# arkworks-rs/sumcheck

Measured on AMD Instinct MI355X. Metric: MLSumcheck prover field-ops/s (BLS12-381 Fr, nv=24), higher is better.
Workload: dtype u256 (BLS12-381 Fr, Montgomery form; integer arithmetic on 9 x 29-bit limbs); 1 GPU; BASELINE config 3: MLSumcheck prove, ListOfProducts [[0, 1, 2, 3], [4, 5, 6], [7, 8], [9]] over 10 tables, nv=24 (24 per GPU shard), BLS12-381 Fr, tables HBM-resident; nv=24, nv_per_gpu=24, tables=10, degree=4, launcher=single process, ranks_seen=1, communicator=none, round_loop=library, round_loop_reason=single GPU: no exchange

## Files before the change

### sumcheck_amd/build.py

```python
from __future__ import annotations

import os
import subprocess
import sys

HERE = os.path.dirname(os.path.abspath(__file__))
CSRC = os.path.join(HERE, "csrc")
OUT = os.path.join(HERE, "libsumcheck_hip.so")
OUT_EXP = os.path.join(HERE, "libsumcheck_hip_exp.so")
SOURCES = ["kernels_big.hip", "kernels_lag.hip", "kernels.hip", "kernels_tail.hip", "kernels_batch.hip", "kernels_batch_gkr.hip", "kernels_batch_eval.hip", "kernels_batch_rounds.hip", "kernels_wide.hip", "kernels_wide16.hip", "gkr.hip", "abi.hip", "protocol.hip", "batch.hip", "batch_rounds.hip", "comm.hip", "kernels_selftest.hip"]
HEADERS = ["fr_device.hpp", "fe_device.hpp", "f29_pack.hpp","kernel_common.hpp", "finalize_device.hpp", "batch_round.hpp", "wide_cell.hpp", "fe_mad_chain.inc", "fr_mac.inc", "fr_mul_gen.inc", "kernels.h", "host_fr.hpp", "transcript.hpp", "prover_internal.hpp", "load_factor.hpp", "wide_tree.hpp", "lag_index.hpp", "lane_sum.hpp", os.path.join("..", "..", "include", "sumcheck_hip.h")]
EXTRA = os.environ.get("SC_BUILD_EXTRA", "").split()
FLAGS = ["--offload-arch=gfx950", "-O3", "-std=c++17", "-fPIC", "-fvisibility=hidden", "-Wall", "-Wno-unused-function"]


def _stale(out: str) -> bool:
    if not os.path.exists(out):
        return True
    t = os.path.getmtime(out)
    deps = [os.path.join(CSRC, s) for s in SOURCES + HEADERS] + [os.path.abspath(__file__)]
    return any(os.path.getmtime(d) > t for d in deps if os.path.exists(d))


def _obj_stale(obj: str, src: str, cmd: list) -> bool:
    dep = obj + ".d"
    if not (os.path.exists(obj) and os.path.exists(dep)):
# ... 89 lines not shown
```

### sumcheck_amd/csrc/abi.hip

```cpp
#include "prover_internal.hpp"

static std::atomic<uint32_t> g_publish_timeout_ms{0};
std::chrono::milliseconds publish_timeout() {
    uint32_t ms = g_publish_timeout_ms.load(std::memory_order_relaxed);
    if (ms == 0) {
        const char *e = std::getenv("SC_PUBLISH_TIMEOUT_MS");
        const long v = e ? std::atol(e) : 0;
        ms = v > 0 ? (uint32_t)std::min<long>(v, 3600 * 1000L) : 20000u;
        g_publish_timeout_ms.store(ms, std::memory_order_relaxed);
    }
    return std::chrono::milliseconds(ms);
}
extern "C" int sc_set_publish_timeout_ms(uint32_t ms) {
    g_publish_timeout_ms.store(ms ? ms : 20000u, std::memory_order_relaxed);
    return SC_OK;
}
static thread_local std::string g_last_error;
static thread_local int g_device = 0;

static std::recursive_mutex g_gate_mutex[64];
thread_local uint16_t g_gate_depth[64];
void gate_lock(int device) {
    g_gate_mutex[(unsigned)device & 63u].lock();
    ++g_gate_depth[(unsigned)device & 63u];
// ... 53 lines not shown

int resident_quiesce(sc_prover *p);
void prover_destroy(sc_prover *p) {
    if (!p) return;
    (void)resident_quiesce(p);
    DeviceGate gate_(p->device);
    (void)hipSetDevice(p->device);
    if (p->deferred_pending && p->sig) {
        __atomic_store_n(p->sig, p->sig_seq, __ATOMIC_RELEASE);
        p->deferred_pending = false;
    }
    if (p->own_stream) (void)hipStreamSynchronize(p->own_stream);
    if (p->arena) (void)hipFree(p->arena);
    if (p->d_partials) (void)hipFree(p->d_partials);
    if (p->d_lag_area) (void)hipFree(p->d_lag_area);
    if (p->d_partials2) (void)hipFree(p->d_partials2);
    if (p->d_fin_counters) (void)hipFree(p->d_fin_counters);
    if (p->d_finprods) (void)hipFree(p->d_finprods);
    if (p->d_W) (void)hipFree(p->d_W);
    if (p->d_scratch) (void)hipFree(p->d_scratch);
    if (p->d_sums[0]) (void)hipFree(p->d_sums[0]);
    if (p->d_out) (void)hipFree(p->d_out);
    if (p->h_out) (void)hipHostFree(p->h_out);
    if (p->h_flag) (void)hipHostFree(p->h_flag);
    for (int q = 0; q < 2; ++q) {
        if (p->ring[q]) (void)hipFree(p->ring[q]);
        if (p->ev_copied[q]) (void)hipEventDestroy(p->ev_copied[q]);
        if (p->ev_consumed[q]) (void)hipEventDestroy(p->ev_consumed[q]);
    }
    if (p->d_chunk_msg) (void)hipFree(p->d_chunk_msg);
// ... 931 lines not shown
        old = g_pool.h;
        g_pool.h = nullptr;
    }
    if (old) prover_destroy(old);
}

namespace {
struct PolicyDef {
    const char *name;
    int64_t def, lo, hi;
};
constexpr PolicyDef kPolicyDefs[scd::kPolCount] = {
    {"pipeline", 1, 0, 1},     {"resident", 1, 0, 1},          {"tail_slices", 1, 0, 1}, {"vram_mailbox", 1, 0, 1},           {"wide_tree", 1, 0, 1},
    {"rccl_direct", 1, 0, 1},  {"shard_gather_log2", 15, 1, 15}, {"gkr_direct", 1, 0, 1},  {"wait_spins", 1 << 22, 1, 0xffffffffLL}, {"tail", 1, 0, 1},
    {"staged_init", 1, 0, 1},  {"batch", 1, 0, 2},        {"lag_single", 2, 0, scd::kLagMaxSkip},
};
struct PolicyTable {
    std::atomic<int64_t> v[scd::kPolCount];
    PolicyTable() {
        for (int i = 0; i < scd::kPolCount; ++i) {
            int64_t x = kPolicyDefs[i].def;
#ifdef SC_EXPERIMENTS
            std::string env = "SC_";
            for (const char *c = kPolicyDefs[i].name; *c; ++c) env += (char)std::toupper((unsigned char)*c);
            if (const char *e = std::getenv(env.c_str())) x = std::min(std::max<int64_t>(std::atoll(e), kPolicyDefs[i].lo), kPolicyDefs[i].hi);
#endif
            v[i].store(x, std::memory_order_relaxed);
        }
    }
};
// ... 288 lines not shown
```

### sumcheck_amd/csrc/kernels.h

```cpp
#pragma once
#include <hip/hip_runtime.h>
#include <stdint.h>

#include "lag_index.hpp"
#include "lane_sum.hpp"

namespace scd {

constexpr int kMaxFusedM = 8;
constexpr int kMaxSmallTables = 32;
constexpr uint64_t kSmallRoundPairs = 1u << 14;

struct FrHost {
    uint64_t l[4];
};

constexpr int32_t kNodeInf = 0x7fffffff;
__host__ __device__ constexpr int32_t node_value(int s) {
    return s == 0 ? 0 : s == 1 ? 1 : s == 2 ? kNodeInf : ((s - 3) % 2 == 0 ? -((s - 3) / 2 + 1) : ((s - 3) / 2 + 2));
}

struct BindConst {
    int32_t R[9][9];
};
// ... 31 lines not shown
    uint64_t w_off[kMaxRoundProds];
    const uint4 *Wm;
    uint4 *partials2;
    uint32_t *counters;
    uint4 *out;
    uint64_t *out_wide;
    uint4 *h_out;
    uint32_t *h_flag;
    uint32_t seq;
};
struct RoundArgs {
    TreeProd prod[kMaxRoundProds];
    int n_prod;
    RoundFin fin;
    uint32_t part_stride, part_block0;
    uint32_t binding;
};

struct FinProd {
    uint32_t M;
    uint32_t pad;
    uint64_t partial_off;
    uint64_t w_off;
};

struct TablePtrs {
    const uint4 *src[kMaxSmallTables];
    uint4 *dst[kMaxSmallTables];
    uint8_t src_f29[kMaxSmallTables];
};
// ... 168 lines not shown

enum PolicyKey {
    kPolPipeline = 0,
    kPolResident,
    kPolTailSlices,
    kPolVramMailbox,
    kPolWideTree,
    kPolRcclDirect,
    kPolShardGatherLog2,
    kPolGkrDirect,
    kPolWaitSpins,
    kPolTail,
    kPolStagedInit,
    kPolBatch,
    kPolLagSingle,
    kPolCount
};
int64_t policy(int key);

enum Plan {
    kPlanBigMergedRound1 = 0,
    kPlanBigMergedBindChain,
    kPlanBigMergedBind,
    kPlanBigClaimIdentity,
    kPlanBigF29Store,
    kPlanBigCanonicalStore,
    kPlanBigPerProductTree,
    kPlanBigWide,
    kPlanBigWide16,
    kPlanBigGeneric,
// ... 127 lines not shown
```

### sumcheck_amd/csrc/kernels_big.hip

```cpp
#include "kernel_common.hpp"
#include "finalize_device.hpp"
#include "load_factor.hpp"

#include <algorithm>
#include <cstdlib>
#include <cstring>

namespace scd {

#ifdef SC_EXPERIMENTS
template <int M>
__global__ __launch_bounds__(kBlock) void k_prod_round(const ProdArgs A, const FrHost r_h, const uint64_t n_pairs,
                                                       uint4 *__restrict__ partials) {
    __shared__ uint32_t sm[kBlock / 64][8];
    const FrU r = fru_from_host(r_h);
    Fr acc[M + 1];
#pragma unroll
    for (int t = 0; t <= M; ++t) acc[t] = fr_zero();

    const uint64_t stride = (uint64_t)gridDim.x * kBlock;
    for (uint64_t b = (uint64_t)blockIdx.x * kBlock + threadIdx.x; b < n_pairs; b += stride) {
        Fr prod[M + 1];
        bool first = true;
        for (int s = 0; s < A.n_slots; ++s) {
// ... 111 lines not shown
        for (int t = 0; t <= M; ++t) acc[t] = fe_carry_pass(fe_add(acc[t], prod[t]));
        if ((iter & 31u) == 31u) {
#pragma unroll
            for (int t = 0; t <= M; ++t) acc[t] = fe_from_fr(fe_to_fr(acc[t]));
        }
    }
#pragma unroll
    for (int t = 0; t <= M; ++t) {
        const Fr s = block_sum(fe_to_fr(acc[t]), sm);
        if (threadIdx.x == 0) fr_store(partials + 2 * ((uint64_t)t * gridDim.x + blockIdx.x), s);
    }
}

template <int M, bool kR1 = false, bool kChain = kChainDefault, bool kSkip1 = false>
__device__ __forceinline__ void tree_pass(const Slot *S, const int32_t (&r)[kBindLds], const uint64_t n_pairs, uint4 *__restrict__ row, uint32_t (*sm)[8],
                                          int32_t *lacc, const uint32_t part_stride = 0, uint4 *__restrict__ lag_area = nullptr, const int lag_m = 0) {
    const uint64_t pstride = part_stride ? part_stride : gridDim.x;
    static_assert(!(kSkip1 && kR1), "round 1 has no previous round to take node 1 from");
    int32_t *my = lacc + threadIdx.x;
#pragma unroll
    for (int i = 0; i < 9 * (M + 1); ++i) my[i * kBlock] = 0;
    const uint64_t stride = (uint64_t)gridDim.x * kBlock;
    uint32_t iter = 0;
    uint64_t b = (uint64_t)blockIdx.x * kBlock + threadIdx.x;
#ifdef SC_M4_PAIRS
    constexpr bool kM4Pairs = true;
#else
    constexpr bool kM4Pairs = kR1;
#endif
    if constexpr (tree_two_pairs(M, kM4Pairs)) {
        for (; b + stride < n_pairs; b += 2 * stride, ++iter) {
            Fe P[M + 1];
            const uint64_t b2 = b + stride;
            [[maybe_unused]] auto accumulate = [&](const int t, const Fe &v) {
                Fe acc;
#pragma unroll
                for (int l = 0; l < 9; ++l) acc.l[l] = my[(9 * t + l) * kBlock];
                acc = fe_add(acc, v);
                if (iter & 1u) acc = fe_carry_pass(acc);
// ... 239 lines not shown
                    x[((wave << lag_m) + (int)lag_class_hi(lane, lag_m)) * 8 + i] = cls[1].v[i];
                }
            }
            __syncthreads();
            if ((int)threadIdx.x < (1 << lag_m)) {
                const int c = threadIdx.x;
                Fr acc;
#pragma unroll
                for (int i = 0; i < 8; ++i) acc.v[i] = x[c * 8 + i];
                for (int w = 1; w < kBlock / 64; ++w) {
                    Fr o;
#pragma unroll
                    for (int i = 0; i < 8; ++i) o.v[i] = x[(((w << lag_m) + c)) * 8 + i];
                    acc = fr_add(acc, o);
                }
                fr_store(lag_area + 2 * ((uint64_t)c * gridDim.x + blockIdx.x), acc);
            }
            __syncthreads();
        }
    }
#else
#pragma unroll
    for (int t = 0; t <= M; ++t) {
        if (kSkip1 && t == 1) continue;
        Fe a;
#pragma unroll
        for (int l = 0; l < 9; ++l) a.l[l] = my[(9 * t + l) * kBlock];
        const Fr s = block_sum(fe_to_fr(a), sm);
        if (threadIdx.x == 0) fr_store(row + 2 * ((uint64_t)t * pstride), s);
    }
#endif
}

template <int M>
__global__ __launch_bounds__(kBlock) void k_prod_tree(const ProdArgs A, const BindConst r, const uint64_t n_pairs,
                                                      uint4 *__restrict__ partials) {
    __shared__ uint32_t sm[kBlock / 64][8];
    __shared__ int32_t rt[kBindLds];
    __shared__ int32_t lacc[9 * (M + 1) * kBlock];
    bind_consts_to_lds(r, rt);
    tree_pass<M>(A.slot, rt, n_pairs, partials + 2 * (uint64_t)blockIdx.x, sm, lacc);
}

#ifdef SC_EXPERIMENTS
constexpr int kTilePairs = 64;

template <int M>
__global__ __launch_bounds__(64 * (M + 1)) void k_round_tile(const ProdArgs A, const FrHost r32_h, const uint64_t n_pairs,
                                                             uint4 *__restrict__ partials) {
    constexpr int kThreads = 64 * (M + 1);
    constexpr int kEnt = 2 * kTilePairs;
    __shared__ int32_t lds[M * 9 * kEnt];
    const FeU r = feu_from_host(r32_h);
    const int tid = threadIdx.x;
    const int node_idx = tid >> 6;
    const int lane = tid & 63;
// ... 74 lines not shown
__global__ __launch_bounds__(kBlock, 3) void k_round_tree(const RoundArgs R, const BindConst r, const uint64_t n_pairs,
                                                       uint4 *__restrict__ partials) {
    __shared__ uint32_t sm[kBlock / 64][8];
    __shared__ int32_t rt[kBindLds];
    __shared__ int32_t lacc[9 * 5 * kBlock];
#ifdef SC_EXPERIMENTS
    __shared__ uint32_t role_sh;
#endif
    bind_consts_to_lds(r, rt);
    const int n = R.n_prod;
    int k = (int)((blockIdx.x & 7u) % (uint32_t)n);
    for (int i = 0; i < n; ++i) {
        const TreeProd &T = R.prod[k];
        uint4 *row = partials + 2 * (T.partial_off + (uint64_t)blockIdx.x);
        switch (T.M) {
        case 1: tree_pass<1>(T.slot, rt, n_pairs, row, sm, lacc); break;
        case 2: tree_pass<2>(T.slot, rt, n_pairs, row, sm, lacc); break;
        case 3: tree_pass<3>(T.slot, rt, n_pairs, row, sm, lacc); break;
        default: tree_pass<4>(T.slot, rt, n_pairs, row, sm, lacc); break;
        }
        if (++k == n) k = 0;
    }
#ifdef SC_EXPERIMENTS
    if (!R.fin.enabled) return;
    const uint32_t G = gridDim.x, n_groups = (G + kFinGroup - 1) / kFinGroup;
    const uint32_t g = blockIdx.x / kFinGroup, g_first = g * kFinGroup, g_size = min((uint32_t)kFinGroup, G - g_first);
    __syncthreads();
    if (threadIdx.x == 0) {
        __builtin_amdgcn_fence(__ATOMIC_RELEASE, "agent");
        const uint32_t d = __hip_atomic_fetch_add(R.fin.counters + 1 + g, 1u, __ATOMIC_RELAXED, __HIP_MEMORY_SCOPE_AGENT);
        role_sh = d == g_size - 1 ? 1u : 0u;
        if (role_sh) __builtin_amdgcn_fence(__ATOMIC_ACQUIRE, "agent");
    }
    __syncthreads();
// ... 28 lines not shown
        __hip_atomic_store(R.fin.counters + i, 0u, __ATOMIC_RELAXED, __HIP_MEMORY_SCOPE_AGENT);
    auto prod_of = [&](int q) -> FinProd {
        FinProd f;
        f.M = R.prod[q].M;
        f.pad = 0;
        f.partial_off = R.prod[q].partial_off;
        f.w_off = R.fin.w_off[q];
        return f;
    };
    finalize_body<kBlock>(prod_of, R.fin.Wm, n, R.fin.D, (int)n_groups, R.fin.partials2, reinterpret_cast<uint4 *>(lacc), R.fin.out, R.fin.out_wide,
                          R.fin.h_out, R.fin.h_flag, R.fin.seq, 1);
#endif
}
#endif

__global__ __launch_bounds__(kBlock, 3) void k_round1_tree_split(const RoundArgs R, const uint64_t n_pairs, uint4 *__restrict__ partials) {
    __shared__ uint32_t sm[kBlock / 64][8];
    __shared__ int32_t rt[kBindLds];
    __shared__ int32_t lacc[9 * 5 * kBlock];
    const TreeProd &T = R.prod[blockIdx.y];
    uint4 *row = partials + 2 * (T.partial_off + (uint64_t)R.part_block0 + (uint64_t)blockIdx.x);
#ifdef SC_NO_CHAIN_R1
    constexpr bool kC1 = false;
#else
    constexpr bool kC1 = true;
#endif
    switch (T.M) {
    case 1: tree_pass<1, true, kC1>(T.slot, rt, n_pairs, row, sm, lacc, R.part_stride, T.slot[0].dst, (int)T.lag_m); break;
    case 2: tree_pass<2, true, kC1>(T.slot, rt, n_pairs, row, sm, lacc, R.part_stride); break;
    case 3: tree_pass<3, true, kC1>(T.slot, rt, n_pairs, row, sm, lacc, R.part_stride); break;
    default: tree_pass<4, true, kC1>(T.slot, rt, n_pairs, row, sm, lacc, R.part_stride); break;
    }
}
template <bool kSkip1>
__device__ __forceinline__ void class_row(const TreeProd &T, const int32_t (&rt)[kBindLds], uint4 *__restrict__ row, uint32_t *x) {
    if (blockIdx.x != 0) {
        if (threadIdx.x == 0) {
            fr_store(row, fr_zero());
            if (!kSkip1) fr_store(row + 2 * (uint64_t)gridDim.x, fr_zero());
        }
        return;
    }
    const int m = (int)T.lag_m, done = (int)T.lag_done;
    const uint32_t G = T.lag_grid;
    uint4 *area = T.slot[0].dst;
    uint4 *tabs = area + 2 * lag_area_partials(m, G);
    const int n_cur = 1 << (m - done);
    if (done == 0) {
        const int per = kBlock >> m, c = (int)threadIdx.x / per, sub = (int)threadIdx.x % per;
        Fr acc = fr_zero();
        for (uint32_t b = (uint32_t)sub; b < G; b += (uint32_t)per) acc = fr_add(acc, fr_load(area + 2 * ((uint64_t)c * G + b)));
        for (int off = per >> 1; off >= 1; off >>= 1) acc = fr_add(acc, fr_shfl_down(acc, off));
        if (sub == 0) {
#pragma unroll
// ... 16 lines not shown
        const Fe l = fe_from_fr(lo), h = fe_from_fr(hi);
        const Fr v = fe_to_fr(fe_add(l, fe_mul_bind<kChainDefault>(fe_sub(h, l), rt)));
        fr_store(tabs + 2 * ((uint64_t)(((done + 1) & 1) << m) + threadIdx.x), v);
#pragma unroll
        for (int i = 0; i < 8; ++i) y[threadIdx.x * 8 + i] = v.v[i];
    }
    __syncthreads();
    if (threadIdx.x < 2 && !(kSkip1 && threadIdx.x == 1)) {
        Fr acc = fr_zero();
        for (int e = (int)threadIdx.x; e < n_cur / 2; e += 2) {
            Fr o;
#pragma unroll
            for (int i = 0; i < 8; ++i) o.v[i] = y[e * 8 + i];
            acc = fr_add(acc, o);
        }
        fr_store(row + 2 * ((uint64_t)threadIdx.x * gridDim.x), acc);
    }
}
template <bool kChain, bool kSkip1, bool kLag = false>
__global__ __launch_bounds__(kBlock, 3) void k_round_tree_split(const RoundArgs R, const BindConst r, const uint64_t n_pairs, uint4 *__restrict__ partials) {
    __shared__ uint32_t sm[kBlock / 64][8];
    __shared__ int32_t rt[kBindLds];
    __shared__ int32_t lacc[9 * 5 * kBlock];
    bind_consts_to_lds(r, rt);
    const TreeProd &T = R.prod[blockIdx.y];
    uint4 *row = partials + 2 * (T.partial_off + (uint64_t)blockIdx.x);
    if constexpr (kLag) {
        if (T.lag_m != 0) {
            class_row<kSkip1>(T, rt, row, reinterpret_cast<uint32_t *>(lacc));
            return;
        }
    }
    switch (T.M) {
    case 1: tree_pass<1, false, kChain, kSkip1>(T.slot, rt, n_pairs, row, sm, lacc); break;
    case 2: tree_pass<2, false, kChain, kSkip1>(T.slot, rt, n_pairs, row, sm, lacc); break;
    case 3: tree_pass<3, false, kChain, kSkip1>(T.slot, rt, n_pairs, row, sm, lacc); break;
    default: tree_pass<4, false, kChain, kSkip1>(T.slot, rt, n_pairs, row, sm, lacc); break;
    }
}

#ifdef SC_EXPERIMENTS
__global__ __launch_bounds__(kBlock, 3) void k_round1_tree(const RoundArgs R, const uint64_t n_pairs, uint4 *__restrict__ partials) {
    __shared__ uint32_t sm[kBlock / 64][8];
    __shared__ int32_t rt[kBindLds];
    __shared__ int32_t lacc[9 * 5 * kBlock];
    const int n = R.n_prod;
    int k = (int)((blockIdx.x & 7u) % (uint32_t)n);
    for (int i = 0; i < n; ++i) {
        const TreeProd &T = R.prod[k];
        uint4 *row = partials + 2 * (T.partial_off + (uint64_t)blockIdx.x);
        switch (T.M) {
        case 1: tree_pass<1, true>(T.slot, rt, n_pairs, row, sm, lacc); break;
        case 2: tree_pass<2, true>(T.slot, rt, n_pairs, row, sm, lacc); break;
        case 3: tree_pass<3, true>(T.slot, rt, n_pairs, row, sm, lacc); break;
        default: tree_pass<4, true>(T.slot, rt, n_pairs, row, sm, lacc); break;
        }
        if (++k == n) k = 0;
    }
}
#endif

#ifdef SC_EXPERIMENTS
template <int M>
static hipError_t launch_prod_round_t(const ProdArgs &args, const FrHost &r, uint64_t n_pairs, FrHost *d_partials, int grid,
                                      hipStream_t stream) {
    hipLaunchKernelGGL(k_prod_round<M>, dim3(grid), dim3(kBlock), 0, stream, args, r, n_pairs, (uint4 *)d_partials);
    return hipGetLastError();
}

#endif
// ... 61 lines not shown
#else
    (void)split;
    (void)extra_lds;
#endif
#ifdef SC_NO_CHAIN_R2
    bool canonical_sources = false;
#else
    bool canonical_sources = !round1;
#endif
    for (int q = 0; q < args.n_prod && canonical_sources; ++q)
        for (uint32_t f = 0; f < args.prod[q].M; ++f) canonical_sources = canonical_sources && args.prod[q].slot[f].src_f29 == 0;
#ifdef SC_SERIAL_EPILOGUE
    for (int q = 0; q < args.n_prod; ++q)
        if (args.prod[q].lag_m != 0) return hipErrorInvalidValue;
#endif
    const dim3 g(grid, args.n_prod), b(kBlock);
    uint4 *const part = (uint4 *)d_partials;
    plan_hit(round1 ? kPlanBigMergedRound1 : canonical_sources ? kPlanBigMergedBindChain : kPlanBigMergedBind);
    if (skip1) plan_hit(kPlanBigClaimIdentity);
    if (round1) {
        if (skip1) return hipErrorInvalidValue;
        hipLaunchKernelGGL(k_round1_tree_split, g, b, 0, stream, args, n_pairs, part);
    } else {
        bool lag = false;
        for (int q = 0; q < args.n_prod; ++q) lag = lag || args.prod[q].lag_m != 0;
        const int sel = (canonical_sources ? 4 : 0) | (skip1 ? 2 : 0) | (lag ? 1 : 0);
        switch (sel) {
        case 7: hipLaunchKernelGGL((k_round_tree_split<true, true, true>), g, b, 0, stream, args, r32, n_pairs, part); break;
        case 6: hipLaunchKernelGGL((k_round_tree_split<true, true, false>), g, b, 0, stream, args, r32, n_pairs, part); break;
        case 5: hipLaunchKernelGGL((k_round_tree_split<true, false, true>), g, b, 0, stream, args, r32, n_pairs, part); break;
        case 4: hipLaunchKernelGGL((k_round_tree_split<true, false, false>), g, b, 0, stream, args, r32, n_pairs, part); break;
// ... 58 lines not shown
```

### sumcheck_amd/csrc/protocol.hip

```cpp
#include "prover_internal.hpp"

uint64_t small_pairs_limit() {
#ifdef SC_EXPERIMENTS
    static const uint64_t v = [] {
        const char *e = std::getenv("SC_SMALL_LOG2");
        return e ? (1ULL << std::atoi(e)) : scd::kSmallRoundPairs;
    }();
    return v;
#else
    return scd::kSmallRoundPairs;
#endif
}

bool launches_are_async(sc_prover *p) {
    static const bool ok = [p] {
        uint32_t *h = nullptr, *d = nullptr;
        FrHost *dm = nullptr;
        if (hipHostMalloc(reinterpret_cast<void **>(&h), 256, hipHostMallocMapped | hipHostMallocCoherent) != hipSuccess) return false;
        bool good = hipHostGetDevicePointer(reinterpret_cast<void **>(&d), h, 0) == hipSuccess &&
                    hipMalloc(reinterpret_cast<void **>(&dm), sizeof(FrHost)) == hipSuccess;
        if (good) {
            std::memset(h, 0, 256);
            good = scd::launch_wait_challenge(d, 0xffffffffu, reinterpret_cast<const FrHost *>(d + 16), dm, p->stream, 1) == hipSuccess &&
                   hipStreamSynchronize(p->stream) == hipSuccess;
// ... 128 lines not shown
        for (uint32_t l = 0; l < k; ++l) make_bind_const(p->lag.r[l], A.r[l]);
        A.levels = k;
        A.n_groups = (1ULL << p->nv) >> 2;
        for (Table &t : p->tabs) {
            if (!t.lag) continue;
            A.src = t.cur;
            A.dst = t.buf[t.next];
            scd::plan_hit(catch_up ? scd::kPlanBigLagCatchUp : scd::kPlanBigLagMaterialize);
            HIP_TRY(scd::launch_fix_deep(A, p->use_f29, p->stream));
            t.cur = t.buf[t.next];
            t.cur_f29 = p->use_f29;
            t.next ^= 1;
        }
    }
    lag_clear(p);
    return SC_OK;
}

int launch_round_streamed(sc_prover *p, const uint64_t *r_or_null, uint64_t *d_wide, bool publish_to_host) {
    scd::plan_hit(scd::kPlanBigStreamed);
    if (p->exhausted) return sc_internal_fail(SC_ERR_NOT_ACTIVE, "Prover is not active");
    if (r_or_null && p->round == 0) return sc_internal_fail(SC_ERR_FIRST_ROUND_HAS_MSG, "first round should be prover first.");
    if (!r_or_null && p->round > 0) return sc_internal_fail(SC_ERR_MISSING_MSG, "verifier message is empty");
    sch::Fr r = sch::zero();
    if (r_or_null) {
        std::memcpy(&r, r_or_null, 32);
        if (sch::geq_p(r)) return sc_internal_fail(SC_ERR_BAD_ARG, "challenge is not a canonical field element");
    }
    HIP_TRY(hipSetDevice(p->device));
    int rc_t = collect_timing(p);
// ... 41 lines not shown
                        sl.src_f29 = 0;
                        if (!bind) {
                            sl.mode = 0;
                        } else if (!bound[u]) {
                            sl.mode = 1;
                            sl.dst = t.buf[0] + 2 * (c * (C / 2));
                            sl.dst_f29 = p->use_f29 ? 1 : 0;
                            bound[u] = 1;
                        } else {
                            sl.mode = 3;
                            sl.dst_f29 = p->use_f29 ? 1 : 0;
                        }
                    }
                }
            }
            HIP_TRY(scd::launch_round_tree(ra, rc, pairs_per_chunk, p->d_partials, grid, p->stream, true));
            if (bind) {
                for (uint32_t u = 0; u < p->U; ++u)
                    if (!bound[u]) HIP_TRY(scd::launch_fix(ring_tab(u), p->tabs[u].buf[0] + 2 * (c * (C / 2)), to_dev(r), C / 2, p->stream));
            }
        } else {
            std::vector<const uint4 *> src(p->U);
            for (uint32_t u = 0; u < p->U; ++u) {
                if (bind) {
                    uint4 *dst = p->tabs[u].buf[0] + 2 * (c * (C / 2));
                    HIP_TRY(scd::launch_fix(ring_tab(u), dst, to_dev(r), C / 2, p->stream));
                    src[u] = dst;
                } else {
                    src[u] = ring_tab(u);
                }
// ... 127 lines not shown
        for (uint32_t k = 0; k < p->K; ++k) {
            const Product &pr = p->prods[k];
            scd::TreeProd &tp = ra.prod[k];
            tp.M = pr.M;
            tp.partial_off = pr.partial_off;
            int f = 0;
            for (size_t s2 = 0; s2 < pr.tables.size(); ++s2)
                for (uint32_t rep = 0; rep < pr.exps[s2]; ++rep, ++f) {
                    tp.slot[f].exp = 1;
                    tp.slot[f].mode = 0;
                    tp.slot[f].src = p->tabs[pr.tables[s2]].buf[0] + 2 * (size_t)first;
                }
        }
        ra.part_stride = (uint32_t)G;
        ra.part_block0 = (uint32_t)block0;
        HIP_TRY(scd::launch_round_tree(ra, rc, chunk >> 1, p->d_partials, gc, p->stream, true, false));
        block0 += gc;
    }
    if (block0 != G) return sc_internal_fail(SC_ERR_HIP, "staged initialisation: the sections do not cover the grid");
    scd::plan_hit(scd::kPlanBigStagedRound1);
    const bool keeps = scd::finalize_keeps_sums((int)p->K, (int)p->D, G, !p->h_finprods.empty(), fin_mb_enabled());
    HIP_TRY(scd::launch_finalize(p->d_finprods, p->h_finprods.data(), p->d_W, (int)p->K, (int)p->D, G, p->d_partials, keeps ? p->d_sums[1] : p->d_scratch, p->d_out, nullptr,
                                 p->h_out_dev, p->h_flag_dev, p->seq + 1, 1, fin_mb_enabled() ? p->d_fin_mb_counter : nullptr, p->stream, nullptr));
    p->r1_cached = true;
    p->r1_keeps = keeps;
    return SC_OK;
}

int launch_round(sc_prover *p, const uint64_t *r_or_null, uint64_t *d_wide, bool publish_to_host, bool deferred) {
    if (p->res.active) {
// ... 291 lines not shown
        }
        p->seq += 1;
        ra.fin.enabled = p->fused_finalize ? 1 : 0;
        ra.fin.D = (int)p->D;
        for (uint32_t k = 0; k < p->K; ++k) ra.fin.w_off[k] = p->h_finprods[k].w_off;
        ra.fin.Wm = reinterpret_cast<const uint4 *>(p->d_W);
        ra.fin.partials2 = reinterpret_cast<uint4 *>(p->d_partials2);
        ra.fin.counters = p->d_fin_counters;
        ra.fin.out = reinterpret_cast<uint4 *>(p->d_out);
        ra.fin.out_wide = d_wide;
        ra.fin.h_out = publish_to_host ? reinterpret_cast<uint4 *>(p->h_out_dev) : nullptr;
        ra.fin.h_flag = publish_to_host ? p->h_flag_dev : nullptr;
        ra.fin.seq = p->seq;
        if (p->timing) HIP_TRY(hipEventRecord(p->prod_ev[0], p->stream));
        if (bind) scd::plan_hit(p->use_f29 ? scd::kPlanBigF29Store : scd::kPlanBigCanonicalStore);
        HIP_TRY(scd::launch_round_tree(ra, rc, n_pairs, p->d_partials, grid, p->stream, split, skip1));
        if (p->timing) HIP_TRY(hipEventRecord(p->prod_ev[1], p->stream));
        scaled = 1;
        if (p->fused_finalize) finalized = true;
        else p->seq -= 1;
    }
    for (uint32_t k = 0; k < p->K && !small && !merged; ++k) {
        const Product &pr = p->prods[k];
        FrHost *partials = p->d_partials + pr.partial_off;
        if (p->timing) HIP_TRY(hipEventRecord(p->prod_ev[2 * k], p->stream));
        if (pr.fused && p->kernel_variant == 3 && (pr.M <= 4 || p->wide_tree)) {
            ProdArgs a;
            std::memset(&a, 0, sizeof(a));
            a.n_slots = (int)pr.M;
            int f = 0;
// ... 990 lines not shown
```

### sumcheck_amd/csrc/prover_internal.hpp

```cpp
#pragma once
#include <hip/hip_runtime.h>

#include <dlfcn.h>
#include <rccl/rccl.h>

#include <algorithm>
#include <array>
#include <atomic>
#include <chrono>
#include <condition_variable>
#include <map>
#include <memory>
#include <mutex>
#include <cstdarg>
#include <cstdio>
#include <cstdlib>
#include <cstring>
#include <new>
#include <string>
#include <thread>
#include <vector>

#include "../../include/sumcheck_hip.h"
#include "host_fr.hpp"
// ... 86 lines not shown
    uint32_t *d_fin_counters = nullptr;
    FinProd *d_finprods = nullptr;
    FrHost *d_W = nullptr;
    uint32_t w_elems = 0;
    bool w_scaled = false;
    FrHost *d_scratch = nullptr;
    FrHost *d_sums[2] = {nullptr, nullptr};
    int64_t sums_round = -1;
    struct Lag {
        bool active = false;
        uint32_t j = 0, m = 0, grid = 0;
        std::vector<sch::Fr> r;
    } lag;
    FrHost *d_lag_area = nullptr;
    uint32_t lag_areas = 0;
    FrHost *d_out = nullptr;
    FrHost *h_out = nullptr;
    uint32_t *h_flag = nullptr;
    FrHost *h_out_dev = nullptr;
    uint32_t *h_flag_dev = nullptr;
    uint32_t seq = 0;
    uint64_t *d_wide = nullptr;
    uint32_t wide_gen = 0;
    bool wide_tagged = false;
    uint64_t *h_wide = nullptr;
    uint64_t *h_wide_dev = nullptr;
    void *d_tail_send = nullptr, *d_tail_recv = nullptr, *d_tail_tabs = nullptr;
    sc_prover *tail = nullptr;
    uint32_t tail_ranks = 0;
    size_t tail_buf_bytes = 0;
// ... 69 lines not shown
bool handle_pool_offer(sc_prover *p);
std::vector<uint8_t> pool_key_of(const sc_poly_desc *d, int device);
sc_prover *handle_pool_take(const std::vector<uint8_t> &key);
void claim_weights(uint32_t M, const sch::Fr &r, sch::Fr *lam);
void build_node_matrix(uint32_t M, uint32_t D, const sch::Fr &scale, std::vector<sch::Fr> &out);
int collect_timing(sc_prover *p);
int prover_bind_out(sc_prover *p, const uint64_t *r, uint64_t *d_out);
uint64_t sc_internal_cache_limit();
constexpr int kResidentGone = -1;
extern std::atomic<uint64_t> g_stat[8];
enum { kStatTailLaunches = 0, kStatTailSlotBusy = 1, kStatTailSlotReclaims = 2, kStatResidentStarts = 3, kStatResidentGone = 4, kStatProofRetries = 5, kStatTailSlices = 6 };
bool wide_tree_enabled();
int resident_quiesce(sc_prover *p);
int launch_round(sc_prover *p, const uint64_t *r_or_null, uint64_t *d_wide, bool publish_to_host, bool deferred = false);
int materialize_lagging(sc_prover *p, bool catch_up = false);
void lag_clear(sc_prover *p);
bool staged_init_applies(const sc_prover *p);
int staged_copy_and_round1(sc_prover *p, const uint64_t *const *host_tables);
int await_round(sc_prover *p, uint64_t *out_evals, uint32_t want);
bool wait_gave_up(sc_prover *p);
void abandon_deferred(sc_prover *p);
int sc_internal_run_rounds(sc_prover *p, sch::Blake2b512Rng &rng, uint32_t n_rounds, uint64_t *out_msgs, sch::Fr *out_challenges);
bool launches_are_async(sc_prover *p);
bool tail_slot_acquire(sc_prover *p, bool resident);
void tail_slot_release(sc_prover *p);
void sc_internal_release_batch_cache();
struct SharedMeta {
    uint32_t nv = 0, U = 0, K = 0, D = 0, max_mult = 0;
    int n_combos = 0;
    bool fits_args = false;
// ... 79 lines not shown
```

Baseline: 559.1 billion field-ops/s.

## Schedule round-tree blocks through a weighted row-order table for load balance

Replaces the 2D grid (blocks × products) of the split tree kernels with a 1D grid that reads a host-built schedule table mapping each block to a (product row, block index). Rows are ranked by estimated multiply/bind cost, and heavier rows are issued earlier by a configurable lead, so long-running product rows start first and the tail of the dispatch is filled with cheaper work. Tables are cached per prover and uploaded once. This adds a table lookup per block and a host build plus copy on first use.

Measured after the change: 561.1 billion field-ops/s, median of 6. No clear change (+0.4%).

```diff
diff --git a/sumcheck_amd/build.py b/sumcheck_amd/build.py
--- a/sumcheck_amd/build.py
+++ b/sumcheck_amd/build.py
@@ -9,7 +9,7 @@
 OUT = os.path.join(HERE, "libsumcheck_hip.so")
 OUT_EXP = os.path.join(HERE, "libsumcheck_hip_exp.so")
 SOURCES = ["kernels_big.hip", "kernels_lag.hip", "kernels.hip", "kernels_tail.hip", "kernels_batch.hip", "kernels_batch_gkr.hip", "kernels_batch_eval.hip", "kernels_batch_rounds.hip", "kernels_wide.hip", "kernels_wide16.hip", "gkr.hip", "abi.hip", "protocol.hip", "batch.hip", "batch_rounds.hip", "comm.hip", "kernels_selftest.hip"]
-HEADERS = ["fr_device.hpp", "fe_device.hpp", "f29_pack.hpp","kernel_common.hpp", "finalize_device.hpp", "batch_round.hpp", "wide_cell.hpp", "fe_mad_chain.inc", "fr_mac.inc", "fr_mul_gen.inc", "kernels.h", "host_fr.hpp", "transcript.hpp", "prover_internal.hpp", "load_factor.hpp", "wide_tree.hpp", "lag_index.hpp", "lane_sum.hpp", os.path.join("..", "..", "include", "sumcheck_hip.h")]
+HEADERS = ["fr_device.hpp", "fe_device.hpp", "f29_pack.hpp","kernel_common.hpp", "finalize_device.hpp", "batch_round.hpp", "wide_cell.hpp", "fe_mad_chain.inc", "fr_mac.inc", "fr_mul_gen.inc", "kernels.h", "host_fr.hpp", "transcript.hpp", "prover_internal.hpp", "load_factor.hpp", "wide_tree.hpp", "lag_index.hpp", "lane_sum.hpp", "row_schedule.hpp", os.path.join("..", "..", "include", "sumcheck_hip.h")]
 EXTRA = os.environ.get("SC_BUILD_EXTRA", "").split()
 FLAGS = ["--offload-arch=gfx950", "-O3", "-std=c++17", "-fPIC", "-fvisibility=hidden", "-Wall", "-Wno-unused-function"]
 
diff --git a/sumcheck_amd/csrc/abi.hip b/sumcheck_amd/csrc/abi.hip
--- a/sumcheck_amd/csrc/abi.hip
+++ b/sumcheck_amd/csrc/abi.hip
@@ -91,6 +91,8 @@
     if (p->arena) (void)hipFree(p->arena);
     if (p->d_partials) (void)hipFree(p->d_partials);
     if (p->d_lag_area) (void)hipFree(p->d_lag_area);
+    for (auto &rs : p->row_scheds)
+        if (rs.d_table) (void)hipFree(rs.d_table);
     if (p->d_partials2) (void)hipFree(p->d_partials2);
     if (p->d_fin_counters) (void)hipFree(p->d_fin_counters);
     if (p->d_finprods) (void)hipFree(p->d_finprods);
@@ -1052,6 +1054,7 @@
     {"pipeline", 1, 0, 1},     {"resident", 1, 0, 1},          {"tail_slices", 1, 0, 1}, {"vram_mailbox", 1, 0, 1},           {"wide_tree", 1, 0, 1},
     {"rccl_direct", 1, 0, 1},  {"shard_gather_log2", 15, 1, 15}, {"gkr_direct", 1, 0, 1},  {"wait_spins", 1 << 22, 1, 0xffffffffLL}, {"tail", 1, 0, 1},
     {"staged_init", 1, 0, 1},  {"batch", 1, 0, 2},        {"lag_single", 2, 0, scd::kLagMaxSkip},
+    {"row_lead_r1", 4, 0, scd::kSchedMaxLead}, {"row_lead", 4, 0, scd::kSchedMaxLead},
 };
 struct PolicyTable {
     std::atomic<int64_t> v[scd::kPolCount];
diff --git a/sumcheck_amd/csrc/kernels.h b/sumcheck_amd/csrc/kernels.h
--- a/sumcheck_amd/csrc/kernels.h
+++ b/sumcheck_amd/csrc/kernels.h
@@ -4,6 +4,7 @@
 
 #include "lag_index.hpp"
 #include "lane_sum.hpp"
+#include "row_schedule.hpp"
 
 namespace scd {
 
@@ -69,6 +70,8 @@
     int n_prod;
     RoundFin fin;
     uint32_t part_stride, part_block0;
+    const uint16_t *sched;
+    uint32_t row_blocks;
     uint32_t binding;
 };
 
@@ -267,6 +270,8 @@
     kPolStagedInit,
     kPolBatch,
     kPolLagSingle,
+    kPolRowLeadR1,
+    kPolRowLead,
     kPolCount
 };
 int64_t policy(int key);
diff --git a/sumcheck_amd/csrc/kernels_big.hip b/sumcheck_amd/csrc/kernels_big.hip
--- a/sumcheck_amd/csrc/kernels_big.hip
+++ b/sumcheck_amd/csrc/kernels_big.hip
@@ -149,15 +149,16 @@
 
 template <int M, bool kR1 = false, bool kChain = kChainDefault, bool kSkip1 = false>
 __device__ __forceinline__ void tree_pass(const Slot *S, const int32_t (&r)[kBindLds], const uint64_t n_pairs, uint4 *__restrict__ row, uint32_t (*sm)[8],
-                                          int32_t *lacc, const uint32_t part_stride = 0, uint4 *__restrict__ lag_area = nullptr, const int lag_m = 0) {
-    const uint64_t pstride = part_stride ? part_stride : gridDim.x;
+                                          int32_t *lacc, const uint32_t bx, const uint32_t nb, const uint32_t part_stride = 0, uint4 *__restrict__ lag_area = nullptr,
+                                          const int lag_m = 0) {
+    const uint64_t pstride = part_stride ? part_stride : nb;
     static_assert(!(kSkip1 && kR1), "round 1 has no previous round to take node 1 from");
     int32_t *my = lacc + threadIdx.x;
 #pragma unroll
     for (int i = 0; i < 9 * (M + 1); ++i) my[i * kBlock] = 0;
-    const uint64_t stride = (uint64_t)gridDim.x * kBlock;
+    const uint64_t stride = (uint64_t)nb * kBlock;
     uint32_t iter = 0;
-    uint64_t b = (uint64_t)blockIdx.x * kBlock + threadIdx.x;
+    uint64_t b = (uint64_t)bx * kBlock + threadIdx.x;
 #ifdef SC_M4_PAIRS
     constexpr bool kM4Pairs = true;
 #else
@@ -427,7 +428,7 @@
                     for (int i = 0; i < 8; ++i) o.v[i] = x[(((w << lag_m) + c)) * 8 + i];
                     acc = fr_add(acc, o);
                 }
-                fr_store(lag_area + 2 * ((uint64_t)c * gridDim.x + blockIdx.x), acc);
+                fr_store(lag_area + 2 * ((uint64_t)c * nb + bx), acc);
             }
             __syncthreads();
         }
@@ -452,7 +453,7 @@
     __shared__ int32_t rt[kBindLds];
     __shared__ int32_t lacc[9 * (M + 1) * kBlock];
     bind_consts_to_lds(r, rt);
-    tree_pass<M>(A.slot, rt, n_pairs, partials + 2 * (uint64_t)blockIdx.x, sm, lacc);
+    tree_pass<M>(A.slot, rt, n_pairs, partials + 2 * (uint64_t)blockIdx.x, sm, lacc, blockIdx.x, gridDim.x);
 }
 
 #ifdef SC_EXPERIMENTS
@@ -557,10 +558,10 @@
         const TreeProd &T = R.prod[k];
         uint4 *row = partials + 2 * (T.partial_off + (uint64_t)blockIdx.x);
         switch (T.M) {
-        case 1: tree_pass<1>(T.slot, rt, n_pairs, row, sm, lacc); break;
-        case 2: tree_pass<2>(T.slot, rt, n_pairs, row, sm, lacc); break;
-        case 3: tree_pass<3>(T.slot, rt, n_pairs, row, sm, lacc); break;
-        default: tree_pass<4>(T.slot, rt, n_pairs, row, sm, lacc); break;
+        case 1: tree_pass<1>(T.slot, rt, n_pairs, row, sm, lacc, blockIdx.x, gridDim.x); break;
+        case 2: tree_pass<2>(T.slot, rt, n_pairs, row, sm, lacc, blockIdx.x, gridDim.x); break;
+        case 3: tree_pass<3>(T.slot, rt, n_pairs, row, sm, lacc, blockIdx.x, gridDim.x); break;
+        default: tree_pass<4>(T.slot, rt, n_pairs, row, sm, lacc, blockIdx.x, gridDim.x); break;
         }
         if (++k == n) k = 0;
     }
@@ -619,30 +620,35 @@
 }
 #endif
 
+__device__ __forceinline__ uint32_t sched_item(const RoundArgs &R) {
+    return sched_entry_of_word(reinterpret_cast<const uint32_t *>(R.sched)[blockIdx.x >> 1], blockIdx.x);
+}
 __global__ __launch_bounds__(kBlock, 3) void k_round1_tree_split(const RoundArgs R, const uint64_t n_pairs, uint4 *__restrict__ partials) {
     __shared__ uint32_t sm[kBlock / 64][8];
     __shared__ int32_t rt[kBindLds];
     __shared__ int32_t lacc[9 * 5 * kBlock];
-    const TreeProd &T = R.prod[blockIdx.y];
-    uint4 *row = partials + 2 * (T.partial_off + (uint64_t)R.part_block0 + (uint64_t)blockIdx.x);
+    const uint32_t item = sched_item(R), nb = R.row_blocks, bx = min(sched_x(item), nb - 1u);
+    const TreeProd &T = R.prod[min(sched_row(item), (uint32_t)R.n_prod - 1u)];
+    uint4 *row = partials + 2 * (T.partial_off + (uint64_t)R.part_block0 + (uint64_t)bx);
 #ifdef SC_NO_CHAIN_R1
     constexpr bool kC1 = false;
 #else
     constexpr bool kC1 = true;
 #endif
     switch (T.M) {
-    case 1: tree_pass<1, true, kC1>(T.slot, rt, n_pairs, row, sm, lacc, R.part_stride, T.slot[0].dst, (int)T.lag_m); break;
-    case 2: tree_pass<2, true, kC1>(T.slot, rt, n_pairs, row, sm, lacc, R.part_stride); break;
-    case 3: tree_pass<3, true, kC1>(T.slot, rt, n_pairs, row, sm, lacc, R.part_stride); break;
-    default: tree_pass<4, true, kC1>(T.slot, rt, n_pairs, row, sm, lacc, R.part_stride); break;
+    case 1: tree_pass<1, true, kC1>(T.slot, rt, n_pairs, row, sm, lacc, bx, nb, R.part_stride, T.slot[0].dst, (int)T.lag_m); break;
+    case 2: tree_pass<2, true, kC1>(T.slot, rt, n_pairs, row, sm, lacc, bx, nb, R.part_stride); break;
+    case 3: tree_pass<3, true, kC1>(T.slot, rt, n_pairs, row, sm, lacc, bx, nb, R.part_stride); break;
+    default: tree_pass<4, true, kC1>(T.slot, rt, n_pairs, row, sm, lacc, bx, nb, R.part_stride); break;
     }
 }
 template <bool kSkip1>
-__device__ __forceinline__ void class_row(const TreeProd &T, const int32_t (&rt)[kBindLds], uint4 *__restrict__ row, uint32_t *x) {
-    if (blockIdx.x != 0) {
+__device__ __forceinline__ void class_row(const TreeProd &T, const int32_t (&rt)[kBindLds], uint4 *__restrict__ row, uint32_t *x, const uint32_t bx,
+                                          const uint32_t nb) {
+    if (bx != 0) {
         if (threadIdx.x == 0) {
             fr_store(row, fr_zero());
-            if (!kSkip1) fr_store(row + 2 * (uint64_t)gridDim.x, fr_zero());
+            if (!kSkip1) fr_store(row + 2 * (uint64_t)nb, fr_zero());
         }
         return;
     }
@@ -689,7 +695,7 @@
             for (int i = 0; i < 8; ++i) o.v[i] = y[e * 8 + i];
             acc = fr_add(acc, o);
         }
-        fr_store(row + 2 * ((uint64_t)threadIdx.x * gridDim.x), acc);
+        fr_store(row + 2 * ((uint64_t)threadIdx.x * nb), acc);
     }
 }
 template <bool kChain, bool kSkip1, bool kLag = false>
@@ -698,19 +704,20 @@
     __shared__ int32_t rt[kBindLds];
     __shared__ int32_t lacc[9 * 5 * kBlock];
     bind_consts_to_lds(r, rt);
-    const TreeProd &T = R.prod[blockIdx.y];
-    uint4 *row = partials + 2 * (T.partial_off + (uint64_t)blockIdx.x);
+    const uint32_t item = sched_item(R), nb = R.row_blocks, bx = min(sched_x(item), nb - 1u);
+    const TreeProd &T = R.prod[min(sched_row(item), (uint32_t)R.n_prod - 1u)];
+    uint4 *row = partials + 2 * (T.partial_off + (uint64_t)bx);
     if constexpr (kLag) {
         if (T.lag_m != 0) {
-            class_row<kSkip1>(T, rt, row, reinterpret_cast<uint32_t *>(lacc));
+            class_row<kSkip1>(T, rt, row, reinterpret_cast<uint32_t *>(lacc), bx, nb);
             return;
         }
     }
     switch (T.M) {
-    case 1: tree_pass<1, false, kChain, kSkip1>(T.slot, rt, n_pairs, row, sm, lacc); break;
-    case 2: tree_pass<2, false, kChain, kSkip1>(T.slot, rt, n_pairs, row, sm, lacc); break;
-    case 3: tree_pass<3, false, kChain, kSkip1>(T.slot, rt, n_pairs, row, sm, lacc); break;
-    default: tree_pass<4, false, kChain, kSkip1>(T.slot, rt, n_pairs, row, sm, lacc); break;
+    case 1: tree_pass<1, false, kChain, kSkip1>(T.slot, rt, n_pairs, row, sm, lacc, bx, nb); break;
+    case 2: tree_pass<2, false, kChain, kSkip1>(T.slot, rt, n_pairs, row, sm, lacc, bx, nb); break;
+    case 3: tree_pass<3, false, kChain, kSkip1>(T.slot, rt, n_pairs, row, sm, lacc, bx, nb); break;
+    default: tree_pass<4, false, kChain, kSkip1>(T.slot, rt, n_pairs, row, sm, lacc, bx, nb); break;
     }
 }
 
@@ -725,10 +732,10 @@
         const TreeProd &T = R.prod[k];
         uint4 *row = partials + 2 * (T.partial_off + (uint64_t)blockIdx.x);
         switch (T.M) {
-        case 1: tree_pass<1, true>(T.slot, rt, n_pairs, row, sm, lacc); break;
-        case 2: tree_pass<2, true>(T.slot, rt, n_pairs, row, sm, lacc); break;
-        case 3: tree_pass<3, true>(T.slot, rt, n_pairs, row, sm, lacc); break;
-        default: tree_pass<4, true>(T.slot, rt, n_pairs, row, sm, lacc); break;
+        case 1: tree_pass<1, true>(T.slot, rt, n_pairs, row, sm, lacc, blockIdx.x, gridDim.x); break;
+        case 2: tree_pass<2, true>(T.slot, rt, n_pairs, row, sm, lacc, blockIdx.x, gridDim.x); break;
+        case 3: tree_pass<3, true>(T.slot, rt, n_pairs, row, sm, lacc, blockIdx.x, gridDim.x); break;
+        default: tree_pass<4, true>(T.slot, rt, n_pairs, row, sm, lacc, blockIdx.x, gridDim.x); break;
         }
         if (++k == n) k = 0;
     }
@@ -820,7 +827,9 @@
     for (int q = 0; q < args.n_prod; ++q)
         if (args.prod[q].lag_m != 0) return hipErrorInvalidValue;
 #endif
-    const dim3 g(grid, args.n_prod), b(kBlock);
+    if (args.sched == nullptr || args.row_blocks != (uint32_t)grid || grid < 1 || grid > kSchedMaxBlocks || args.n_prod < 1 || args.n_prod > kSchedMaxRows)
+        return hipErrorInvalidValue;
+    const dim3 g((uint32_t)grid * (uint32_t)args.n_prod), b(kBlock);
     uint4 *const part = (uint4 *)d_partials;
     plan_hit(round1 ? kPlanBigMergedRound1 : canonical_sources ? kPlanBigMergedBindChain : kPlanBigMergedBind);
     if (skip1) plan_hit(kPlanBigClaimIdentity);
diff --git a/sumcheck_amd/csrc/protocol.hip b/sumcheck_amd/csrc/protocol.hip
--- a/sumcheck_amd/csrc/protocol.hip
+++ b/sumcheck_amd/csrc/protocol.hip
@@ -166,6 +166,39 @@
         }
     }
     lag_clear(p);
+    return SC_OK;
+}
+
+int prover_row_schedule(sc_prover *p, scd::RoundArgs &ra, int grid, int lead, bool skip1) {
+    const int K = ra.n_prod;
+    if (K < 1 || K > scd::kSchedMaxRows || grid < 1 || grid > scd::kSchedMaxBlocks) return sc_internal_fail(SC_ERR_HIP, "no block schedule for %d rows of %d blocks", K, grid);
+    lead = std::min(std::max(lead, 0), scd::kSchedMaxLead);
+    uint32_t w[scd::kSchedMaxRows] = {};
+    for (int q = 0; q < K; ++q) {
+        const scd::TreeProd &T = ra.prod[q];
+        int binds = 0;
+        for (uint32_t f = 0; f < T.M; ++f) binds += T.slot[f].mode != 0 ? 1 : 0;
+        w[q] = scd::sched_row_weight((int)T.M, skip1, binds, ra.binding != 0 && T.lag_m != 0);
+    }
+    ra.row_blocks = (uint32_t)grid;
+    for (const sc_prover::RowSched &rs : p->row_scheds)
+        if (rs.K == (uint32_t)K && rs.g == (uint32_t)grid && rs.lead == (uint32_t)lead && std::memcmp(rs.weight, w, sizeof(w)) == 0) {
+            ra.sched = rs.d_table;
+            return SC_OK;
+        }
+    std::vector<uint16_t> h(2 * (size_t)scd::sched_table_words(K, grid), 0);
+    if (scd::sched_build(w, K, grid, lead, h.data()) != (uint32_t)K * (uint32_t)grid) return sc_internal_fail(SC_ERR_HIP, "the block schedule was not built");
+    sc_prover::RowSched rs;
+    rs.K = (uint32_t)K, rs.g = (uint32_t)grid, rs.lead = (uint32_t)lead;
+    std::memcpy(rs.weight, w, sizeof(w));
+    HIP_TRY(hipMalloc(reinterpret_cast<void **>(&rs.d_table), h.size() * sizeof(uint16_t)));
+    const hipError_t e = hipMemcpy(rs.d_table, h.data(), h.size() * sizeof(uint16_t), hipMemcpyHostToDevice);
+    if (e != hipSuccess) {
+        (void)hipFree(rs.d_table);
+        HIP_TRY(e);
+    }
+    p->row_scheds.push_back(rs);
+    ra.sched = rs.d_table;
     return SC_OK;
 }
 
@@ -237,6 +270,7 @@
                     }
                 }
             }
+            if (int rc_s = prover_row_schedule(p, ra, grid, (int)scd::policy(bind ? scd::kPolRowLead : scd::kPolRowLeadR1), false)) return rc_s;
             HIP_TRY(scd::launch_round_tree(ra, rc, pairs_per_chunk, p->d_partials, grid, p->stream, true));
             if (bind) {
                 for (uint32_t u = 0; u < p->U; ++u)
@@ -394,6 +428,7 @@
         }
         ra.part_stride = (uint32_t)G;
         ra.part_block0 = (uint32_t)block0;
+        if (int rc_s = prover_row_schedule(p, ra, gc, scd::kSchedMaxLead, false)) return rc_s;
         HIP_TRY(scd::launch_round_tree(ra, rc, chunk >> 1, p->d_partials, gc, p->stream, true, false));
         block0 += gc;
     }
@@ -715,6 +750,8 @@
         ra.fin.seq = p->seq;
         if (p->timing) HIP_TRY(hipEventRecord(p->prod_ev[0], p->stream));
         if (bind) scd::plan_hit(p->use_f29 ? scd::kPlanBigF29Store : scd::kPlanBigCanonicalStore);
+        if (split)
+            if (int rc_s = prover_row_schedule(p, ra, grid, (int)scd::policy(bind ? scd::kPolRowLead : scd::kPolRowLeadR1), skip1)) return rc_s;
         HIP_TRY(scd::launch_round_tree(ra, rc, n_pairs, p->d_partials, grid, p->stream, split, skip1));
         if (p->timing) HIP_TRY(hipEventRecord(p->prod_ev[1], p->stream));
         scaled = 1;
diff --git a/sumcheck_amd/csrc/prover_internal.hpp b/sumcheck_amd/csrc/prover_internal.hpp
--- a/sumcheck_amd/csrc/prover_internal.hpp
+++ b/sumcheck_amd/csrc/prover_internal.hpp
@@ -124,6 +124,12 @@
     } lag;
     FrHost *d_lag_area = nullptr;
     uint32_t lag_areas = 0;
+    struct RowSched {
+        uint32_t K = 0, g = 0, lead = 0;
+        uint32_t weight[scd::kSchedMaxRows] = {};
+        uint16_t *d_table = nullptr;
+    };
+    std::vector<RowSched> row_scheds;
     FrHost *d_out = nullptr;
     FrHost *h_out = nullptr;
     uint32_t *h_flag = nullptr;
@@ -223,6 +229,7 @@
 int resident_quiesce(sc_prover *p);
 int launch_round(sc_prover *p, const uint64_t *r_or_null, uint64_t *d_wide, bool publish_to_host, bool deferred = false);
 int materialize_lagging(sc_prover *p, bool catch_up = false);
+int prover_row_schedule(sc_prover *p, scd::RoundArgs &ra, int grid, int lead, bool skip1);
 void lag_clear(sc_prover *p);
 bool staged_init_applies(const sc_prover *p);
 int staged_copy_and_round1(sc_prover *p, const uint64_t *const *host_tables);
diff --git a/sumcheck_amd/csrc/row_schedule.hpp b/sumcheck_amd/csrc/row_schedule.hpp
--- /dev/null
+++ b/sumcheck_amd/csrc/row_schedule.hpp
@@ -0,0 +1,64 @@
+#pragma once
+#include <cstdint>
+
+#if defined(__HIPCC__)
+#define SC_SCHED_FN __host__ __device__ constexpr
+#else
+#define SC_SCHED_FN constexpr
+#endif
+
+namespace scd {
+
+constexpr int kSchedMaxRows = 12;
+constexpr int kSchedMaxBlocks = 1024;
+constexpr int kSchedMaxLead = 4;
+constexpr int kSchedXBits = 10;
+constexpr uint32_t kSchedMulMads = 153, kSchedBindMads = 97;
+
+SC_SCHED_FN uint16_t sched_entry(uint32_t row, uint32_t x) { return (uint16_t)((row << kSchedXBits) | x); }
+SC_SCHED_FN uint32_t sched_row(uint32_t entry) { return entry >> kSchedXBits; }
+SC_SCHED_FN uint32_t sched_x(uint32_t entry) { return entry & ((1u << kSchedXBits) - 1u); }
+SC_SCHED_FN uint32_t sched_entry_of_word(uint32_t word, uint32_t i) { return (word >> (16u * (i & 1u))) & 0xffffu; }
+SC_SCHED_FN uint32_t sched_table_words(int K, int g) { return ((uint32_t)K * (uint32_t)g + 1u) / 2u; }
+
+SC_SCHED_FN uint32_t sched_tree_products(int M, bool skip1) {
+    const uint32_t full = M <= 1 ? 0u : M == 2 ? 3u : M == 3 ? 7u : 11u;
+    return full != 0 && skip1 ? full - 1u : full;
+}
+SC_SCHED_FN uint32_t sched_row_weight(int M, bool skip1, int bind_factors, bool class_row) {
+    return class_row ? 0u : kSchedMulMads * sched_tree_products(M, skip1) + kSchedBindMads * 2u * (uint32_t)bind_factors;
+}
+
+SC_SCHED_FN void sched_rank_rows(const uint32_t *weight, int K, uint8_t *rank) {
+    for (int a = 0; a < K; ++a) {
+        int before = 0;
+        for (int b = 0; b < K; ++b)
+            if (weight[b] > weight[a] || (weight[b] == weight[a] && b < a)) ++before;
+        rank[a] = (uint8_t)before;
+    }
+}
+
+SC_SCHED_FN uint32_t sched_key(uint32_t rank, uint32_t x, int g, int lead) { return 4u * x + (uint32_t)lead * rank * (uint32_t)g; }
+
+SC_SCHED_FN uint32_t sched_build(const uint32_t *weight, int K, int g, int lead, uint16_t *out) {
+    if (K < 1 || K > kSchedMaxRows || g < 1 || g > kSchedMaxBlocks || lead < 0 || lead > kSchedMaxLead) return 0;
+    uint8_t rank[kSchedMaxRows] = {};
+    uint32_t row_of[kSchedMaxRows] = {}, next[kSchedMaxRows] = {};
+    sched_rank_rows(weight, K, rank);
+    for (int a = 0; a < K; ++a) row_of[rank[a]] = (uint32_t)a;
+    const uint32_t total = (uint32_t)K * (uint32_t)g;
+    for (uint32_t i = 0; i < total; ++i) {
+        int best = -1;
+        uint32_t best_key = 0;
+        for (int q = 0; q < K; ++q) {
+            if (next[q] == (uint32_t)g) continue;
+            const uint32_t key = sched_key((uint32_t)q, next[q], g, lead);
+            if (best < 0 || key < best_key) best = q, best_key = key;
+        }
+        out[i] = sched_entry(row_of[best], next[best]);
+        ++next[best];
+    }
+    return total;
+}
+
+}
```
